# Hawkeye-FineGrained/Hawkeye

Hardware: NVIDIA H100
Metric: 448x448 images/sec, BCNN VGG-16 train step (fwd+CE+bwd+grad all-reduce+SGD), device-timed, max over ranks (higher is better)
Workload: dtype tf32 (fp32 storage, fp32 accumulate)

## Files before the change

hawkeye_b200/csrc/conv.cu:

```cuda
#include <stdlib.h>

#include "common.cuh"
#include "host.h"
#include "gemm.h"
#include "../../include/hawkeye_b200.h"

namespace hk {

__global__ void pack_weights_kernel(const float* __restrict__ W, float* __restrict__ Wf, float* __restrict__ Wd,
                                    int Cout, int Cin, int round) {
  const size_t n = (size_t)Cout * Cin * 9;
  for (size_t i = blockIdx.x * (size_t)blockDim.x + threadIdx.x; i < n; i += (size_t)gridDim.x * blockDim.x) {
    const int t = i % 9;
    const int ci = (i / 9) % Cin;
    const int co = i / ((size_t)9 * Cin);
    const float v = round ? tf32_round(W[i]) : W[i];
    if (Wf) Wf[((size_t)t * Cout + co) * Cin + ci] = v;
    if (Wd) Wd[((size_t)(8 - t) * Cin + ci) * Cout + co] = v;
  }
}
__global__ void unpack_wgrad_kernel(const float* __restrict__ dWp, float* __restrict__ dW, int Cout, int Cin, int accumulate) {
  const size_t n = (size_t)Cout * Cin * 9;
  for (size_t i = blockIdx.x * (size_t)blockDim.x + threadIdx.x; i < n; i += (size_t)gridDim.x * blockDim.x) {
    const int t = i % 9;
// ... 183 lines not shown
  const int co0 = blockIdx.y * BN;
  const int nchunk = a.Cin / 32;
  const int nk = 9 * nchunk;

  if (threadIdx.x == 0) {
    tma_prefetch_desc(&tmX);
    tma_prefetch_desc(&tmW);
    for (int s = 0; s < Cfg::STAGES; ++s) { mbar_init(&full[s], 1); mbar_init(&empty[s], 2); }
    fence_barrier_init();
  }
  __syncthreads();

  if (warp < 4) {
    regs_dealloc<56>();
    if (threadIdx.x == 0) {
      for (int kb = 0; kb < nk; ++kb) {
        const int s = kb % Cfg::STAGES;
        const uint32_t ph = (kb / Cfg::STAGES) & 1;
        const int tap = kb / nchunk, ck = kb - tap * nchunk;
        const int kh = tap / 3, kw = tap - kh * 3;
        mbar_wait(&empty[s], ph ^ 1);
        mbar_expect_tx(&full[s], Cfg::STAGE_BYTES);
        tma_load_4d(sA + s * Cfg::A_BYTES, &tmX, &full[s], ck * 32, w0 * a.stride + kw - 1, h0 * a.stride + kh - 1, n0);
        tma_load_3d(sB + s * Cfg::B_BYTES, &tmW, &full[s], ck * 32, co0, tap);
      }
    }
  } else {
    regs_alloc<224>();
    const int ct = threadIdx.x - 128;
    const int wg = ct >> 7;
    float acc[NACC];
    for (int kb = 0; kb < nk; ++kb) {
      const int s = kb % Cfg::STAGES;
      const uint32_t ph = (kb / Cfg::STAGES) & 1;
      mbar_wait(&full[s], ph);
      const uint64_t a_base = make_sdesc(smem_u32(sA + s * Cfg::A_BYTES + wg * 64 * 128));
      const uint64_t b_base = make_sdesc(smem_u32(sB + s * Cfg::B_BYTES));
      wgmma_fence();
#pragma unroll
      for (int ks = 0; ks < 4; ++ks) wgmma_tf32(acc, a_base + ks * 2, b_base + ks * 2, (kb | ks) != 0);
      wgmma_commit();
      wgmma_wait<1>();
      wgmma_keep(acc);
      if (kb > 0 && (ct & 127) == 0) mbar_arrive(&empty[(kb - 1) % Cfg::STAGES]);
    }
    wgmma_wait<0>();
    wgmma_keep(acc);
    conv_epilogue<BN>(a, acc, acc_tile, w0, h0, n0, co0, ct);
  }
}

static void pick_tile(int W, int H, int N, int target, int* TW, int* TH, int* TN) {
  int tw = 1;
  while (tw * 2 <= 16 && W % (tw * 2) == 0 && tw * 2 <= target) tw *= 2;
  int th = 1;
  while (th * 2 * tw <= target && H % (th * 2) == 0) th *= 2;
  int tn = target / (tw * th);
  *TW = tw; *TH = th; *TN = tn;
  (void)N;
}

static int make_act_map(CUtensorMap* tm, const float* X, int N, int H, int W, int C, int TW, int TH, int TN,
                        int stride = 1) {
  uint64_t dims[4] = {(uint64_t)C, (uint64_t)W, (uint64_t)H, (uint64_t)N};
  uint64_t strides[3] = {(uint64_t)C * 4, (uint64_t)W * C * 4, (uint64_t)H * W * C * 4};
  uint32_t box[4] = {32, (uint32_t)(TW * stride), (uint32_t)(TH * stride), (uint32_t)TN};
  uint32_t estr[4] = {1, (uint32_t)stride, (uint32_t)stride, 1};
  return make_tmap(tm, X, 4, dims, strides, box, stride > 1 ? estr : nullptr);
}

template <int BN>
static int launch_conv(const CUtensorMap& tmX, const CUtensorMap& tmW, const ConvArgs& a, cudaStream_t stream) {
  using Cfg = ConvCfg<BN>;
  if (int r = allow_dynamic_smem<conv3x3_igemm_kernel<BN>>(Cfg::SMEM, BN == 64 ? "conv<64>" : "conv<128>")) return r;
  dim3 grid(a.tiles_w * a.tiles_h * a.tiles_n, (a.Cout + BN - 1) / BN);
  conv3x3_igemm_kernel<BN><<<grid, CONV_THREADS, Cfg::SMEM, stream>>>(tmX, tmW, a);
  HK_LAUNCH_CHECK("conv3x3_igemm_kernel");
  return 0;
}

constexpr int CONV_V2_THREADS = 512;

enum { EPI_MAP = 0, EPI_UNPOOL = 1, EPI_FIRST_WGRAD = 2 };
constexpr int FW_HALO = 3 * 10 * 18;
constexpr int FW_HALO_BYTES = 2 * FW_HALO * 4;
struct FirstWgradArgs {
  const float* img;
  float* part;
};

__device__ __forceinline__ void mma_m16n8k8_tf32(float (&d)[4], const uint32_t (&a)[4], uint32_t b0, uint32_t b1) {
  asm volatile("mma.sync.aligned.m16n8k8.row.col.f32.tf32.tf32.f32 {%0, %1, %2, %3}, {%4, %5, %6, %7}, {%8, %9}, "
               "{%0, %1, %2, %3};\n"
               : "+f"(d[0]), "+f"(d[1]), "+f"(d[2]), "+f"(d[3])
               : "r"(a[0]), "r"(a[1]), "r"(a[2]), "r"(a[3]), "r"(b0), "r"(b1));
}

template <int BN, bool RESIDENT>
struct ConvV2Cfg {
  static constexpr int A_BYTES = 160 * 128;
  static constexpr int B_TILE = BN * 128;
  static constexpr int STAGE_BYTES = A_BYTES + (RESIDENT ? 0 : 3 * B_TILE);
  static constexpr int STAGES = RESIDENT ? 2 : (BN == 64 ? 3 : 2);
  static constexpr int WRES_BYTES = RESIDENT ? 18 * B_TILE : 0;
  static constexpr int PIECES = STAGES == 2 && !RESIDENT ? 3 : 1;
  static constexpr int STG_LD = BN + 8;
  static constexpr int STG_BYTES = 128 * STG_LD * 4;
  static constexpr int SMEM = STAGES * STAGE_BYTES + WRES_BYTES + 1024 + 256 + STG_BYTES;
};

template <int BN, bool RESIDENT, int TW, int EPI>
__global__ void __launch_bounds__(CONV_V2_THREADS, 1)
conv3x3_igemm_v2_kernel(const __grid_constant__ CUtensorMap tmX, const __grid_constant__ CUtensorMap tmW, ConvArgs a,
                        int n_ntiles, int total_tiles, FirstWgradArgs fw) {
  using Cfg = ConvV2Cfg<BN, RESIDENT>;
  static_assert(EPI != EPI_FIRST_WGRAD || (BN == 64 && RESIDENT && TW == 16), "conv1_1 weight gradient: 64 -> 64, 16 x 8");
  constexpr int NACC = BN / 2;
  constexpr int TN = 16 / TW;
  constexpr int WG_ROWS = TW == 16 ? 64 : 80;
  extern __shared__ uint8_t smem_raw[];
  uint8_t* smem = reinterpret_cast<uint8_t*>((reinterpret_cast<uintptr_t>(smem_raw) + 1023) & ~uintptr_t(1023));
  uint8_t* stages = smem;
  uint8_t* wres = smem + Cfg::STAGES * Cfg::STAGE_BYTES;
  uint64_t* full = reinterpret_cast<uint64_t*>(wres + Cfg::WRES_BYTES);
  uint64_t* empty = full + Cfg::STAGES * Cfg::PIECES;
  uint64_t* wbar = empty + Cfg::STAGES;
  uint64_t* stg_full = wbar + 1;
  uint64_t* stg_empty = wbar + 2;
  float* stg = reinterpret_cast<float*>(wres + Cfg::WRES_BYTES + 256);

  const int warp = threadIdx.x >> 5;
  const int nchunk = a.Cin / 32;
  const int nkb = nchunk * 3;

  if (threadIdx.x == 0) {
    tma_prefetch_desc(&tmX);
    tma_prefetch_desc(&tmW);
    for (int s = 0; s < Cfg::STAGES; ++s) mbar_init(&empty[s], 2);
    for (int i = 0; i < Cfg::STAGES * Cfg::PIECES; ++i) mbar_init(&full[i], 1);
    mbar_init(wbar, 1);
    mbar_init(stg_full, 256);
    mbar_init(stg_empty, 128);
    fence_barrier_init();
  }
  __syncthreads();

  if (warp >= 12 && EPI == EPI_MAP && a.P) {
    const int r = threadIdx.x - 384;
    int j = 0;
    for (int t = blockIdx.x; t < total_tiles; t += gridDim.x, ++j) {
      int pt = t / n_ntiles;
      const int co0 = (t - pt * n_ntiles) * BN;
      const int tw = pt % a.tiles_w; pt /= a.tiles_w;
      const int th = pt % a.tiles_h; pt /= a.tiles_h;
      mbar_wait(stg_full, j & 1);
      const int w = tw * TW + (r & (TW - 1)), h = th * 8 + ((r / TW) & 7), n = pt * TN + r / (TW * 8);
      const bool valid = TN == 1 || n < a.N;
      const size_t pix = ((size_t)n * a.H + h) * a.W + w;
#pragma unroll 1
      for (int c = 0; c < BN / 32; ++c) {
        float v[32];
        const float4* src = reinterpret_cast<const float4*>(stg + r * Cfg::STG_LD + c * 32);
#pragma unroll
        for (int k = 0; k < 8; ++k) {
          const float4 q = src[k];
          v[4 * k] = q.x; v[4 * k + 1] = q.y; v[4 * k + 2] = q.z; v[4 * k + 3] = q.w;
        }
        if (c == BN / 32 - 1) mbar_arrive(stg_empty);
        epi_chunk<true>(a, v, w, h, n, pix, co0 + c * 32, valid);
      }
    }
  } else if (warp >= 12) {
    const int e = threadIdx.x - 384;
    const int ew = e >> 5, sub = (e >> 3) & 3, u4 = (e & 7) * 4;
    const int p0 = ew * 32 + sub;
    const int eoff0 = (TW == 16 ? (p0 >> 4) * a.W + (p0 & 15) : ((p0 >> 6) * a.H + ((p0 >> 3) & 7)) * a.W + (p0 & 7)) * a.Cout + u4;
    const int erow = a.W * a.Cout, e4 = 4 * a.Cout;
    auto eoff = [&](int k) { return eoff0 + (k / (TW / 4)) * erow + (k % (TW / 4)) * e4; };
    const float* srow = stg + (ew * 32 + sub) * Cfg::STG_LD + u4;
    auto tile_org = [&](int t, size_t& org, int& co0) {
      co0 = (t % n_ntiles) * BN;
      int pt = t / n_ntiles;
      const int tw = pt % a.tiles_w; pt /= a.tiles_w;
      const int th = pt % a.tiles_h; pt /= a.tiles_h;
      org = (((size_t)pt * TN * a.H + th * 8) * a.W + tw * TW) * a.Cout;
      return pt * TN + (TW == 16 ? 0 : ew >> 1) < a.N;
    };
    auto tile_pos = [&](int t, int& tw, int& th, int& tn) {
      int pt = t / n_ntiles;
      tw = pt % a.tiles_w; pt /= a.tiles_w;
      th = pt % a.tiles_h; tn = pt / a.tiles_h;
    };
    const int frow = 2 * a.W * a.Cout;
    const int uoff0 = (TW == 16 ? 2 * (p0 >> 4) * frow + 2 * (p0 & 15) * a.Cout
                                : ((p0 >> 6) * 2 * a.H + 2 * ((p0 >> 3) & 7)) * frow + 2 * (p0 & 7) * a.Cout) + u4;
    auto uoff = [&](int k) { return uoff0 + (k / (TW / 4)) * 2 * frow + (k % (TW / 4)) * 8 * a.Cout; };
    float* halo = stg + 128 * Cfg::STG_LD;
    float dacc[4][4] = {};
    const int lane = e & 31, g = lane >> 2, tq = lane & 3;
    int hoff[4];
#pragma unroll
    for (int nt = 0; nt < 4; ++nt) {
      const int jj = 8 * nt + g;
      hoff[nt] = jj < 27 ? (jj / 9) * 180 + (jj % 9 / 3) * 18 + jj % 3 : 0;
    }
    int co0 = 0, j = 0;
    size_t org = 0;
    for (int t = blockIdx.x; t < total_tiles; t += gridDim.x, ++j) {
      const bool valid = tile_org(t, org, co0);
      if constexpr (EPI == EPI_FIRST_WGRAD) {
        int tw, th, tn;
        tile_pos(t, tw, th, tn);
        float* hb = halo + (j & 1) * FW_HALO;
        for (int i = e; i < FW_HALO; i += 128) {
          const int ci = i / 180, hh = th * 8 - 1 + i / 18 % 10, ww = tw * 16 - 1 + i % 18;
          hb[i] = hh >= 0 && hh < a.H && ww >= 0 && ww < a.W
                      ? tf32_round(__ldg(fw.img + (((size_t)tn * 3 + ci) * a.H + hh) * a.W + ww)) : 0.f;
        }
      }
      mbar_wait(stg_full, j & 1);
#pragma unroll
      for (int c = 0; c < BN / 32; ++c) {
        float4 v[8];
#pragma unroll
        for (int k = 0; k < 8; ++k) v[k] = *reinterpret_cast<const float4*>(srow + 4 * k * Cfg::STG_LD + c * 32);
        if (EPI != EPI_FIRST_WGRAD && c == BN / 32 - 1) mbar_arrive(stg_empty);
        const int co = co0 + c * 32;
        const bool live = valid && co < a.Cout;
        if (live) {
          if (a.bias) {
            const float4 b = __ldg(reinterpret_cast<const float4*>(a.bias + co + u4));
#pragma unroll
            for (int k = 0; k < 8; ++k) { v[k].x += b.x; v[k].y += b.y; v[k].z += b.z; v[k].w += b.w; }
          }
          if (a.relu) {
#pragma unroll
            for (int k = 0; k < 8; ++k) {
              v[k].x = fmaxf(v[k].x, 0.f); v[k].y = fmaxf(v[k].y, 0.f);
              v[k].z = fmaxf(v[k].z, 0.f); v[k].w = fmaxf(v[k].w, 0.f);
            }
          }
          if (a.mask) {
            float4 mk[8];
#pragma unroll
            for (int k = 0; k < 8; ++k) mk[k] = __ldcs(reinterpret_cast<const float4*>(a.mask + org + co + eoff(k)));
#pragma unroll
            for (int k = 0; k < 8; ++k) {
              v[k].x = mk[k].x > 0.f ? v[k].x : 0.f; v[k].y = mk[k].y > 0.f ? v[k].y : 0.f;
              v[k].z = mk[k].z > 0.f ? v[k].z : 0.f; v[k].w = mk[k].w > 0.f ? v[k].w : 0.f;
            }
          }
          if constexpr (EPI == EPI_MAP) {
#pragma unroll
            for (int k = 0; k < 8; ++k)
              __stcs(reinterpret_cast<float4*>(a.Y + org + co + eoff(k)),
                     make_float4(tf32_round(v[k].x), tf32_round(v[k].y), tf32_round(v[k].z), tf32_round(v[k].w)));
          } else if constexpr (EPI == EPI_UNPOOL) {
            int tw, th, tn;
            tile_pos(t, tw, th, tn);
            float* dst = a.Y + (((size_t)tn * TN * 2 * a.H + th * 16) * 2 * a.W + tw * 2 * TW) * a.Cout + co;
            uint32_t cd[8];
#pragma unroll
            for (int k = 0; k < 8; ++k) cd[k] = __ldcs(reinterpret_cast<const unsigned int*>(a.code + org + co + eoff(k)));
#pragma unroll
            for (int k = 0; k < 8; ++k) {
              const float4 q = make_float4((cd[k] & 4u) ? tf32_round(v[k].x) : 0.f, (cd[k] & (4u << 8)) ? tf32_round(v[k].y) : 0.f,
                                           (cd[k] & (4u << 16)) ? tf32_round(v[k].z) : 0.f,
                                           (cd[k] & (4u << 24)) ? tf32_round(v[k].w) : 0.f);
              float* o = dst + uoff(k);
#pragma unroll
              for (int pos = 0; pos < 4; ++pos)
                __stcs(reinterpret_cast<float4*>(o + (pos >> 1) * frow + (pos & 1) * a.Cout),
                       make_float4((cd[k] & 3u) == (uint32_t)pos ? q.x : 0.f, (cd[k] >> 8 & 3u) == (uint32_t)pos ? q.y : 0.f,
                                   (cd[k] >> 16 & 3u) == (uint32_t)pos ? q.z : 0.f,
                                   (cd[k] >> 24 & 3u) == (uint32_t)pos ? q.w : 0.f));
            }
          } else {
#pragma unroll
            for (int k = 0; k < 8; ++k)
              *reinterpret_cast<float4*>(stg + (ew * 32 + sub + 4 * k) * Cfg::STG_LD + u4 + c * 32) =
                  make_float4(tf32_round(v[k].x), tf32_round(v[k].y), tf32_round(v[k].z), tf32_round(v[k].w));
          }
        }
      }
      if constexpr (EPI == EPI_FIRST_WGRAD) {
        named_bar(1, 128);
        const float* hb = halo + (j & 1) * FW_HALO;
        const float* arow = stg + tq * Cfg::STG_LD + 16 * ew + g;
#pragma unroll 4
        for (int ks = 0; ks < 16; ++ks) {
          const float* ap = arow + 8 * ks * Cfg::STG_LD;
          const uint32_t af[4] = {__float_as_uint(ap[0]), __float_as_uint(ap[8]), __float_as_uint(ap[4 * Cfg::STG_LD]),
                                  __float_as_uint(ap[4 * Cfg::STG_LD + 8])};
          const int hp = (ks >> 1) * 18 + 8 * (ks & 1) + tq;
#pragma unroll
          for (int nt = 0; nt < 4; ++nt) {
            float b0 = hb[hoff[nt] + hp], b1 = hb[hoff[nt] + hp + 4];
            if (nt == 3 && g >= 3) b0 = b1 = g == 3 ? 1.f : 0.f;
            mma_m16n8k8_tf32(dacc[nt], af, __float_as_uint(b0), __float_as_uint(b1));
          }
        }
        mbar_arrive(stg_empty);
      }
    }
    if constexpr (EPI == EPI_FIRST_WGRAD) {
      float* dst = fw.part + (size_t)blockIdx.x * 64 * 32;
#pragma unroll
      for (int nt = 0; nt < 4; ++nt)
#pragma unroll
        for (int i = 0; i < 4; ++i) dst[(16 * ew + g + 8 * (i >> 1)) * 32 + 8 * nt + 2 * tq + (i & 1)] = dacc[nt][i];
    }
  } else if (warp < 4) {
    if (threadIdx.x == 0) {
      if (RESIDENT) {
        mbar_expect_tx(wbar, Cfg::WRES_BYTES);
        for (int tap = 0; tap < 9; ++tap)
          for (int ck = 0; ck < 2; ++ck) tma_load_3d(wres + (tap * 2 + ck) * Cfg::B_TILE, &tmW, wbar, ck * 32, 0, tap);
      }
      int kbg = 0;
      for (int t = blockIdx.x; t < total_tiles; t += gridDim.x) {
        const int nt = t % n_ntiles;
        int pt = t / n_ntiles;
        const int tw = pt % a.tiles_w; pt /= a.tiles_w;
        const int th = pt % a.tiles_h; pt /= a.tiles_h;
        const int w0 = tw * TW, h0 = th * 8, n0 = pt * TN, co0 = nt * BN;
        for (int kb = 0; kb < nkb; ++kb, ++kbg) {
          const int s = kbg % Cfg::STAGES;
          const uint32_t ph = (kbg / Cfg::STAGES) & 1;
          const int ck = kb / 3, kw = kb - ck * 3;
          mbar_wait(&empty[s], ph ^ 1);
          uint64_t* f = full + s * Cfg::PIECES;
          uint8_t* st = stages + s * Cfg::STAGE_BYTES;
          mbar_expect_tx(&f[0], Cfg::PIECES == 3 ? Cfg::A_BYTES + Cfg::B_TILE : Cfg::STAGE_BYTES);
          tma_load_4d(st, &tmX, &f[0], ck * 32, w0 + kw - 1, h0 - 1, n0);
          if (!RESIDENT) {
#pragma unroll
            for (int kh = 0; kh < 3; ++kh) {
              uint64_t* fk = &f[Cfg::PIECES == 3 ? kh : 0];
              if (Cfg::PIECES == 3 && kh > 0) mbar_expect_tx(fk, Cfg::B_TILE);
              tma_load_3d(st + Cfg::A_BYTES + kh * Cfg::B_TILE, &tmW, fk, ck * 32, co0, kh * 3 + kw);
            }
          }
        }
      }
    }
  } else {
    const int ct = threadIdx.x - 128;
    const int wg = ct >> 7;
    if (RESIDENT) mbar_wait(wbar, 0);
    float acc[NACC];
#pragma unroll
    for (int i = 0; i < NACC; ++i) acc[i] = 0.f;
    float* frag = stg + (wg * 64 + ((ct >> 5) & 3) * 16 + ((ct & 31) >> 2)) * Cfg::STG_LD + 2 * (ct & 3);
    int kbg = 0, j = 0;
    for (int t = blockIdx.x; t < total_tiles; t += gridDim.x, ++j) {
      for (int kb = 0; kb < nkb; ++kb, ++kbg) {
        const int s = kbg % Cfg::STAGES;
        const int ck = kb / 3, kw = kb - ck * 3;
        const uint32_t ph = (kbg / Cfg::STAGES) & 1;
        const uint32_t a_addr = smem_u32(stages + s * Cfg::STAGE_BYTES) + wg * WG_ROWS * 128;
#pragma unroll
        for (int kh = 0; kh < 3; ++kh) {
          if (kh < Cfg::PIECES) {
            mbar_wait(&full[s * Cfg::PIECES + kh], ph);
            wgmma_fence();
          }
          const uint32_t b_addr = RESIDENT ? smem_u32(wres + ((kh * 3 + kw) * 2 + ck) * Cfg::B_TILE)
                                           : smem_u32(stages + s * Cfg::STAGE_BYTES + Cfg::A_BYTES + kh * Cfg::B_TILE);
          const uint64_t ad = make_sdesc(a_addr + kh * TW * 128), bd = make_sdesc(b_addr);
#pragma unroll
          for (int ks = 0; ks < 4; ++ks) wgmma_tf32(acc, ad + ks * 2, bd + ks * 2, (kb | kh | ks) != 0);
          if (kh >= 3 - Cfg::PIECES) wgmma_commit();
          if (kh == 3 - Cfg::PIECES) {
            wgmma_wait<1>();
            wgmma_keep(acc);
            if (kb > 0 && (ct & 127) == 0) mbar_arrive(&empty[(kbg - 1) % Cfg::STAGES]);
          }
        }
      }
      wgmma_wait<0>();
      wgmma_keep(acc);
      if ((ct & 127) == 0) mbar_arrive(&empty[(kbg - 1) % Cfg::STAGES]);
      mbar_wait(stg_empty, (j & 1) ^ 1);
#pragma unroll
      for (int i = 0; i < NACC / 4; ++i) {
        *reinterpret_cast<float2*>(frag + 8 * i) = make_float2(acc[4 * i], acc[4 * i + 1]);
        *reinterpret_cast<float2*>(frag + 8 * Cfg::STG_LD + 8 * i) = make_float2(acc[4 * i + 2], acc[4 * i + 3]);
      }
      mbar_arrive(stg_full);
    }
  }
}

template <int BN, bool RESIDENT, int TW, int EPI = EPI_MAP>
static int launch_conv_v2(const float* x, const float* wp, ConvArgs a, int N, int H, int W, cudaStream_t stream,
                          FirstWgradArgs fw = {}) {
  using Cfg = ConvV2Cfg<BN, RESIDENT>;
  constexpr int SMEM = Cfg::SMEM + (EPI == EPI_FIRST_WGRAD ? FW_HALO_BYTES : 0);
  static_assert(SMEM <= 232448, "conv_v2: dynamic shared memory above the sm_90 opt-in limit");
  if (int r = allow_dynamic_smem<conv3x3_igemm_v2_kernel<BN, RESIDENT, TW, EPI>>(SMEM, BN == 64 ? "conv_v2<64>" : "conv_v2<128>"))
    return r;
  a.TW = TW; a.TH = 8; a.TN = 16 / TW;
  a.tiles_w = W / TW; a.tiles_h = H / 8; a.tiles_n = (N + a.TN - 1) / a.TN;
  const int n_ntiles = (a.Cout + BN - 1) / BN;
  const long long total = (long long)a.tiles_w * a.tiles_h * a.tiles_n * n_ntiles;
  HK_REQUIRE(total < (1ll << 31), HK_ERR_UNSUPPORTED, "conv3x3: too many tiles");
  HK_REQUIRE((long long)H * W * a.Cout < (1ll << 30), HK_ERR_UNSUPPORTED, "conv3x3: map too large");
  CUtensorMap tmX, tmW;
  int r;
  {
    uint64_t dims[4] = {(uint64_t)a.Cin, (uint64_t)W, (uint64_t)H, (uint64_t)N};
    uint64_t strides[3] = {(uint64_t)a.Cin * 4, (uint64_t)W * a.Cin * 4, (uint64_t)H * W * a.Cin * 4};
    uint32_t box[4] = {32, (uint32_t)TW, 10, (uint32_t)a.TN};
    if ((r = make_tmap(&tmX, x, 4, dims, strides, box))) return r;
  }
  {
    uint64_t dims[3] = {(uint64_t)a.Cin, (uint64_t)a.Cout, 9};
    uint64_t strides[2] = {(uint64_t)a.Cin * 4, (uint64_t)a.Cin * a.Cout * 4};
    uint32_t box[3] = {32, (uint32_t)BN, 1};
    if ((r = make_tmap(&tmW, wp, 3, dims, strides, box))) return r;
  }
  const int sms = num_sms();
  const int grid = total < sms ? (int)total : sms;
  conv3x3_igemm_v2_kernel<BN, RESIDENT, TW, EPI><<<grid, CONV_V2_THREADS, SMEM, stream>>>(tmX, tmW, a, n_ntiles, (int)total, fw);
  HK_LAUNCH_CHECK("conv3x3_igemm_v2_kernel");
  return 0;
}

template <int TW, int EPI = EPI_MAP>
static int launch_conv_v2(const float* x, const float* wp, const ConvArgs& a, int N, int H, int W, cudaStream_t stream) {
  if (a.Cin == 64 && a.Cout == 64) return launch_conv_v2<64, true, TW, EPI>(x, wp, a, N, H, W, stream);
  if (a.Cout <= 64) return launch_conv_v2<64, false, TW, EPI>(x, wp, a, N, H, W, stream);
  return launch_conv_v2<128, false, TW, EPI>(x, wp, a, N, H, W, stream);
}

static int conv3x3_igemm_1x(const float* x, const float* wp, const float* bias, const float* mask, const float* addend,
                            float* y, int N, int H, int W, int Cin, int Cout, int relu, cudaStream_t stream, int stride,
                            int no_round, float* pooled = nullptr, unsigned char* code = nullptr,
                            int pool_nchw = 0);

int conv3x3_igemm(const float* x, const float* wp, const float* bias, const float* mask, float* y, int N, int H, int W,
                  int Cin, int Cout, int relu, cudaStream_t stream, int stride = 1) {
  if (!precise()) return conv3x3_igemm_1x(x, wp, bias, mask, nullptr, y, N, H, W, Cin, Cout, relu, stream, stride, 0);
  HK_REQUIRE(x && wp && y, HK_ERR_ARG, "conv3x3: null pointer");
  const size_t nx = (size_t)N * H * W * Cin, nw = (size_t)9 * Cout * Cin;
  Scratch sx(2 * nx * sizeof(float), stream), sw(2 * nw * sizeof(float), stream);
  HK_REQUIRE(sx.p && sw.p, HK_ERR_DRIVER, "conv3x3 (precise): cudaMallocAsync of the operand halves failed");
  float *xh = sx.f(), *xl = xh + nx, *wh = sw.f(), *wl = wh + nw;
  int r;
  if ((r = tf32_split(x, xh, xl, nx, stream))) return r;
  if ((r = tf32_split(wp, wh, wl, nw, stream))) return r;
  if ((r = conv3x3_igemm_1x(xh, wl, nullptr, nullptr, nullptr, y, N, H, W, Cin, Cout, 0, stream, stride, 1))) return r;
  if ((r = conv3x3_igemm_1x(xl, wh, nullptr, nullptr, y, y, N, H, W, Cin, Cout, 0, stream, stride, 1))) return r;
  return conv3x3_igemm_1x(xh, wh, bias, mask, y, y, N, H, W, Cin, Cout, relu, stream, stride, 1);
}

static int conv3x3_igemm_1x(const float* x, const float* wp, const float* bias, const float* mask, const float* addend,
                            float* y, int N, int H, int W, int Cin, int Cout, int relu, cudaStream_t stream, int stride,
                            int no_round, float* pooled, unsigned char* code, int pool_nchw) {
  const int Hin = H, Win = W;
  if (stride == 2) {
    HK_REQUIRE(H % 2 == 0 && W % 2 == 0, HK_ERR_UNSUPPORTED, "conv3x3 stride 2: even H/W required");
    H /= 2; W /= 2;
  }
  HK_REQUIRE(x && wp && (y || pooled), HK_ERR_ARG, "conv3x3: null pointer");
  HK_REQUIRE(Cin % 32 == 0 && Cout % 32 == 0, HK_ERR_UNSUPPORTED, "conv3x3: Cin=%d Cout=%d must be multiples of 32",
             Cin, Cout);
  HK_REQUIRE(aligned16(x) && aligned16(wp) && (!y || aligned16(y)) && (!mask || aligned16(mask)), HK_ERR_ALIGN,
             "conv3x3: pointer not 16-byte aligned");
  if (pooled)
    HK_REQUIRE(stride == 1 && H % 2 == 0 && W % 2 == 0 && aligned16(pooled) && (!code || aligned16(code)), HK_ERR_UNSUPPORTED,
               "conv3x3 + pool: even H/W, stride 1 and 16-byte aligned outputs required");
  ConvArgs a = {};
  a.P = pooled; a.code = code; a.pool_nchw = pool_nchw;
  a.Y = y; a.bias = bias; a.mask = mask; a.N = N; a.H = H; a.W = W; a.Cin = Cin; a.Cout = Cout; a.relu = relu;
  a.stride = stride;
  a.addend = addend; a.no_round = no_round;
  if (!no_round && stride == 1 && W % 8 == 0 && H % 8 == 0) {
    if (W % 16 == 0) return launch_conv_v2<16>(x, wp, a, N, H, W, stream);
    return launch_conv_v2<8>(x, wp, a, N, H, W, stream);
  }
  pick_tile(W, H, N, 128, &a.TW, &a.TH, &a.TN);
  HK_REQUIRE(!pooled || (a.TW >= 2 && a.TH >= 2), HK_ERR_UNSUPPORTED, "conv3x3 + pool: pixel tile %dx%d", a.TW, a.TH);
  a.tiles_w = (W + a.TW - 1) / a.TW; a.tiles_h = (H + a.TH - 1) / a.TH; a.tiles_n = (N + a.TN - 1) / a.TN;
  HK_REQUIRE((long long)a.tiles_w * a.tiles_h * a.tiles_n < (1ll << 31), HK_ERR_UNSUPPORTED, "conv3x3: grid too large");
  CUtensorMap tmX, tmW;
  int r;
  if ((r = make_act_map(&tmX, x, N, Hin, Win, Cin, a.TW, a.TH, a.TN, stride))) return r;
  const int BN = Cout <= 64 ? 64 : 128;
  {
    uint64_t dims[3] = {(uint64_t)Cin, (uint64_t)Cout, 9};
    uint64_t strides[2] = {(uint64_t)Cin * 4, (uint64_t)Cin * Cout * 4};
    uint32_t box[3] = {32, (uint32_t)BN, 1};
    if ((r = make_tmap(&tmW, wp, 3, dims, strides, box))) return r;
  }
  if (BN == 64) return launch_conv<64>(tmX, tmW, a, stream);
  return launch_conv<128>(tmX, tmW, a, stream);
}

struct WgradArgs {
  float* dWp;
  float* db;
  int N, H, W, Cin, Cout;
  int TW, TH, TN, tiles_w, tiles_h, tiles_n;
  int total_tiles, per;
};

constexpr int WG_THREADS = 4 * 128;
constexpr int WG_PRODUCER_REGS = 56, WG_CONSUMER_REGS = 152;
static_assert(128 * WG_PRODUCER_REGS + 3 * 128 * WG_CONSUMER_REGS <= 65536, "wgrad register budget");
constexpr int WG_STAGES = 3;
constexpr int WG_KP = 64;
constexpr int WG_RAW_ROWS = 120;
constexpr int WG_RAW_BYTES = WG_RAW_ROWS * 128;
// ... 569 lines not shown
  if (sub >= lanes_per_c) return;
  const size_t per = (npix + gridDim.x - 1) / gridDim.x;
  const size_t p0 = blockIdx.x * per, p1 = (p0 + per < npix) ? p0 + per : npix;
  for (int cc = c; cc < C; cc += (blockDim.x < C ? blockDim.x : C)) {
    float s = 0.f;
    for (size_t p = p0 + sub; p < p1; p += lanes_per_c) s += dy[p * C + cc];
    atomicAdd(db + cc, s);
  }
}

}

using namespace hk;

extern "C" {

int hk_conv3x3_pack_weights(const float* w, float* w_fwd, float* w_dgrad, int Cout, int Cin, void* stream) {
  HK_REQUIRE(w && (w_fwd || w_dgrad), HK_ERR_ARG, "hk_conv3x3_pack_weights: null pointer");
  pack_weights_kernel<<<grid_1d((size_t)Cout * Cin * 9, 256), 256, 0, (cudaStream_t)stream>>>(w, w_fwd, w_dgrad, Cout, Cin,
                                                                                              precise() ? 0 : 1);
  HK_LAUNCH_CHECK("pack_weights_kernel");
  return 0;
}

int hk_conv3x3_fwd(const float* x, const float* w_packed, const float* bias, float* y, int N, int H, int W, int Cin,
                   int Cout, int relu, void* stream) {
  return conv3x3_igemm(x, w_packed, bias, nullptr, y, N, H, W, Cin, Cout, relu, (cudaStream_t)stream);
}

int hk_conv3x3_fwd_pool(const float* x, const float* w_packed, const float* bias, float* pooled, unsigned char* code, int N,
                        int H, int W, int Cin, int Cout, int out_nchw, void* stream) {
  HK_REQUIRE(!precise(), HK_ERR_UNSUPPORTED, "hk_conv3x3_fwd_pool: not available in 3xTF32 mode (use conv + pool)");
  HK_REQUIRE(pooled, HK_ERR_ARG, "hk_conv3x3_fwd_pool: null output");
  return conv3x3_igemm_1x(x, w_packed, bias, nullptr, nullptr, nullptr, N, H, W, Cin, Cout, 1, (cudaStream_t)stream, 1,
                          0, pooled, code, out_nchw);
}

int hk_conv3x3_s2_fwd(const float* x, const float* w_packed, const float* bias, float* y, int N, int H, int W, int Cin,
                      int Cout, int relu, void* stream) {
  return conv3x3_igemm(x, w_packed, bias, nullptr, y, N, H, W, Cin, Cout, relu, (cudaStream_t)stream, 2);
}

int hk_conv3x3_dgrad(const float* dy, const float* w_dgrad_packed, const float* relu_mask_act, float* dx, int N, int H,
                     int W, int Cin, int Cout, void* stream) {
  return conv3x3_igemm(dy, w_dgrad_packed, nullptr, relu_mask_act, dx, N, H, W, Cout, Cin, 0, (cudaStream_t)stream);
}

int hk_conv3x3_dgrad_unpool(const float* dy, const float* w_dgrad_packed, const unsigned char* code, float* dx_full, int N,
                            int H, int W, int Cin, int Cout, void* stream) {
  HK_REQUIRE(!precise(), HK_ERR_UNSUPPORTED, "hk_conv3x3_dgrad_unpool: not available in 3xTF32 mode");
  HK_REQUIRE(dy && w_dgrad_packed && code && dx_full, HK_ERR_ARG, "hk_conv3x3_dgrad_unpool: null pointer");
  HK_REQUIRE(N > 0 && H > 0 && W > 0, HK_ERR_ARG, "hk_conv3x3_dgrad_unpool: empty map");
  HK_REQUIRE(Cin % 32 == 0 && Cout % 32 == 0, HK_ERR_UNSUPPORTED,
             "hk_conv3x3_dgrad_unpool: Cin=%d Cout=%d must be multiples of 32", Cin, Cout);
  HK_REQUIRE(H % 8 == 0 && W % 8 == 0, HK_ERR_UNSUPPORTED, "hk_conv3x3_dgrad_unpool: %dx%d map is not a multiple of 8x8",
             H, W);
  HK_REQUIRE(4ll * H * W * Cin < (1ll << 31), HK_ERR_UNSUPPORTED, "hk_conv3x3_dgrad_unpool: map too large");
  HK_REQUIRE(aligned16(dy) && aligned16(w_dgrad_packed) && aligned16(code) && aligned16(dx_full), HK_ERR_ALIGN,
             "hk_conv3x3_dgrad_unpool: pointer not 16-byte aligned");
  ConvArgs a = {};
  a.Y = dx_full; a.code = const_cast<unsigned char*>(code);
  a.N = N; a.H = H; a.W = W; a.Cin = Cout; a.Cout = Cin; a.stride = 1;
  if (W % 16 == 0) return launch_conv_v2<16, EPI_UNPOOL>(dy, w_dgrad_packed, a, N, H, W, (cudaStream_t)stream);
  return launch_conv_v2<8, EPI_UNPOOL>(dy, w_dgrad_packed, a, N, H, W, (cudaStream_t)stream);
}

size_t hk_conv3x3_dgrad_first_wgrad_workspace_bytes(void) { return (size_t)num_sms() * 64 * 32 * sizeof(float); }

int hk_conv3x3_dgrad_first_wgrad_acc(const float* dy, const float* w_dgrad_packed, const float* relu_mask_act,
                                     const float* x_nchw, float* dw1, float* db1, int N, int H, int W, int Cin, int Cout,
                                     void* workspace, size_t workspace_bytes, int accumulate, void* stream_) {
  cudaStream_t stream = (cudaStream_t)stream_;
  HK_REQUIRE(!precise(), HK_ERR_UNSUPPORTED, "hk_conv3x3_dgrad_first_wgrad: not available in 3xTF32 mode");
  HK_REQUIRE(dy && w_dgrad_packed && x_nchw && dw1, HK_ERR_ARG, "hk_conv3x3_dgrad_first_wgrad: null pointer");
  HK_REQUIRE(N > 0 && H > 0 && W > 0, HK_ERR_ARG, "hk_conv3x3_dgrad_first_wgrad: empty map");
  HK_REQUIRE(Cin == 64 && Cout == 64, HK_ERR_UNSUPPORTED, "hk_conv3x3_dgrad_first_wgrad: Cin=%d Cout=%d (64 -> 64 only)",
             Cin, Cout);
  HK_REQUIRE(W % 16 == 0 && H % 8 == 0, HK_ERR_UNSUPPORTED,
             "hk_conv3x3_dgrad_first_wgrad: %dx%d map is not tiled by 16x8", H, W);
  HK_REQUIRE(aligned16(dy) && aligned16(w_dgrad_packed) && (!relu_mask_act || aligned16(relu_mask_act)), HK_ERR_ALIGN,
             "hk_conv3x3_dgrad_first_wgrad: pointer not 16-byte aligned");
  HK_REQUIRE(workspace && workspace_bytes >= hk_conv3x3_dgrad_first_wgrad_workspace_bytes(), HK_ERR_WORKSPACE,
             "hk_conv3x3_dgrad_first_wgrad: workspace too small");
  const long long tiles = (long long)(W / 16) * (H / 8) * N;
  HK_REQUIRE(tiles < (1ll << 31), HK_ERR_UNSUPPORTED, "hk_conv3x3_dgrad_first_wgrad: too many tiles");
  float* part = static_cast<float*>(workspace);
  ConvArgs a = {};
  a.mask = relu_mask_act;
  a.N = N; a.H = H; a.W = W; a.Cin = Cout; a.Cout = Cin; a.stride = 1;
  int r = launch_conv_v2<64, true, 16, EPI_FIRST_WGRAD>(dy, w_dgrad_packed, a, N, H, W, stream, FirstWgradArgs{x_nchw, part});
  if (r) return r;
  const int G = tiles < num_sms() ? (int)tiles : num_sms();
  if ((r = sum_splits(part, G, 64 * 32, 64, 27, 32, dw1, 27, nullptr, accumulate, stream))) return r;
  if (!db1) return 0;
  return sum_splits(part + 27, G, 64 * 32, 64, 1, 32, db1, 1, nullptr, accumulate, stream);
}

size_t hk_conv3x3_wgrad_workspace_bytes(int Cin, int Cout) { return (size_t)9 * Cin * Cout * sizeof(float); }

int hk_conv3x3_wgrad_acc(const float* x, const float* dy, float* dw, float* db, int N, int H, int W, int Cin, int Cout,
                         void* workspace, size_t workspace_bytes, int accumulate, void* stream_) {
  cudaStream_t stream = (cudaStream_t)stream_;
  HK_REQUIRE(workspace && workspace_bytes >= hk_conv3x3_wgrad_workspace_bytes(Cin, Cout), HK_ERR_WORKSPACE,
             "hk_conv3x3_wgrad: workspace too small");
  HK_REQUIRE(dw, HK_ERR_ARG, "hk_conv3x3_wgrad: null dw");
  float* dwp = static_cast<float*>(workspace);
  int r = conv3x3_wgrad(x, dy, dwp, db, N, H, W, Cin, Cout, stream, !accumulate);
  if (r) return r;
  unpack_wgrad_kernel<<<grid_1d((size_t)Cout * Cin * 9, 256), 256, 0, stream>>>(dwp, dw, Cout, Cin, accumulate ? 1 : 0);
  HK_LAUNCH_CHECK("unpack_wgrad_kernel");
  return 0;
}

int hk_conv3x3_wgrad(const float* x, const float* dy, float* dw, float* db, int N, int H, int W, int Cin, int Cout,
                     void* workspace, size_t workspace_bytes, void* stream_) {
  return hk_conv3x3_wgrad_acc(x, dy, dw, db, N, H, W, Cin, Cout, workspace, workspace_bytes, 0, stream_);
}

size_t hk_conv3x3_first_fwd_workspace_bytes(int N, int H, int W, int Cout) {
  return ((size_t)N * H * W * 32 + (size_t)Cout * 32) * sizeof(float);
}

int hk_conv3x3_first_fwd(const float* x_nchw, const float* w, const float* bias, float* y_nhwc, int N, int H, int W,
                         int Cout, void* workspace, size_t workspace_bytes, void* stream_) {
  cudaStream_t stream = (cudaStream_t)stream_;
  HK_REQUIRE(x_nchw && w && y_nhwc, HK_ERR_ARG, "hk_conv3x3_first_fwd: null pointer");
  HK_REQUIRE(Cout % 4 == 0 && Cout <= 256, HK_ERR_UNSUPPORTED, "hk_conv3x3_first_fwd: Cout=%d unsupported", Cout);
  HK_REQUIRE(workspace && workspace_bytes >= hk_conv3x3_first_fwd_workspace_bytes(N, H, W, Cout), HK_ERR_WORKSPACE,
             "hk_conv3x3_first_fwd: workspace too small");
  const long long P = (long long)N * H * W;
  HK_REQUIRE(P < (1ll << 31), HK_ERR_UNSUPPORTED, "hk_conv3x3_first_fwd: too many pixels");
  float* x27 = static_cast<float*>(workspace);
  float* w27 = x27 + (size_t)P * 32;
  const int round = precise() ? 0 : 1;
  im2col_first_kernel<<<grid_1d((size_t)P, 128), 128, 0, stream>>>(x_nchw, x27, N, H, W, round);
  HK_LAUNCH_CHECK("im2col_first_kernel");
  pack_first_weights_kernel<<<(Cout * 32 + 127) / 128, 128, 0, stream>>>(w, bias, w27, Cout, round);
  HK_LAUNCH_CHECK("pack_first_weights_kernel");
  GemmEpi e = {};
  e.C = y_nhwc; e.ldc = Cout; e.alpha = 1.f;
  e.relu = 3;
  return gemm_tf32(x27, 0, 32, 0, w27, 0, 32, 0, e, (int)P, Cout, 32, 1, stream);
}

static int first_wgrad_splits(long long P) {
  for (int S = 592; S > 1; --S)
    if (P % S == 0) return S;
  return 1;
}

size_t hk_conv3x3_first_wgrad_workspace_bytes(int N, int H, int W, int Cout) {
  return (size_t)first_wgrad_splits((long long)N * H * W) * Cout * 32 * sizeof(float);
}

int hk_conv3x3_first_wgrad_acc(const float* x27, const float* dy_nhwc, float* dw, float* db, int N, int H, int W, int Cout,
                               void* workspace, size_t workspace_bytes, int accumulate, void* stream_);
int hk_conv3x3_first_wgrad(const float* x27, const float* dy_nhwc, float* dw, float* db, int N, int H, int W,
                           int Cout, void* workspace, size_t workspace_bytes, void* stream_) {
  return hk_conv3x3_first_wgrad_acc(x27, dy_nhwc, dw, db, N, H, W, Cout, workspace, workspace_bytes, 0, stream_);
}
int hk_conv3x3_first_wgrad_acc(const float* x27, const float* dy_nhwc, float* dw, float* db, int N, int H, int W, int Cout,
                               void* workspace, size_t workspace_bytes, int accumulate, void* stream_) {
  cudaStream_t stream = (cudaStream_t)stream_;
  HK_REQUIRE(x27 && dy_nhwc && dw, HK_ERR_ARG, "hk_conv3x3_first_wgrad: null pointer");
  HK_REQUIRE(Cout % 4 == 0 && Cout <= 128, HK_ERR_UNSUPPORTED, "hk_conv3x3_first_wgrad: Cout=%d unsupported", Cout);
  HK_REQUIRE(workspace && workspace_bytes >= hk_conv3x3_first_wgrad_workspace_bytes(N, H, W, Cout), HK_ERR_WORKSPACE,
             "hk_conv3x3_first_wgrad: workspace too small");
  const long long P = (long long)N * H * W;
  const int S = first_wgrad_splits(P);
  float* part = static_cast<float*>(workspace);
  int r = gemm_splitk(dy_nhwc, 1, Cout, x27, 1, 32, Cout, 32, P, S, part, dw, 27, 27, nullptr, accumulate, stream);
  if (r || !db) return r;
  return sum_splits(part + 27, S, (long long)Cout * 32, Cout, 1, 32, db, 1, nullptr, accumulate, stream);
// ... 83 lines not shown
```

Baseline: 826.7.

## Use 16x16 pixel tiles with swapped wgmma operands for 64-channel TW=16 convs

For BN=64 with 16-wide tiles, the conv kernel now processes a 16x16 (256-pixel) tile by swapping operands so the weights become the wgmma A operand and pixels the N dimension. It streams weights instead of keeping them resident, uses two stages, enlarges the halo and staging buffer, and runs the epilogue in two 128-pixel halves. The first-layer fused dgrad+wgrad path is moved onto this larger tile. The aim is to halve per-tile overhead and halo reloads and to use wider wgmma instructions, at the cost of more shared memory, a transposed staging write pattern with more bank traffic, and handling partial tiles when H is not a multiple of 16.

```diff
diff --git a/hawkeye_b200/csrc/conv.cu b/hawkeye_b200/csrc/conv.cu
--- a/hawkeye_b200/csrc/conv.cu
+++ b/hawkeye_b200/csrc/conv.cu
@@ -289,7 +289,8 @@
 constexpr int CONV_V2_THREADS = 512;
 
 enum { EPI_MAP = 0, EPI_UNPOOL = 1, EPI_FIRST_WGRAD = 2 };
-constexpr int FW_HALO = 3 * 10 * 18;
+constexpr int FW_HALO_CH = 18 * 18;
+constexpr int FW_HALO = 3 * FW_HALO_CH;
 constexpr int FW_HALO_BYTES = 2 * FW_HALO * 4;
 struct FirstWgradArgs {
   const float* img;
@@ -303,16 +304,21 @@
                : "r"(a[0]), "r"(a[1]), "r"(a[2]), "r"(a[3]), "r"(b0), "r"(b1));
 }
 
-template <int BN, bool RESIDENT>
+template <int BN, bool RESIDENT, int TW>
 struct ConvV2Cfg {
-  static constexpr int A_BYTES = 160 * 128;
+  static constexpr bool SWAP = BN == 64 && TW == 16;
+  static_assert(!(SWAP && RESIDENT), "the 256-pixel tile streams its weights");
+  static constexpr int TH = SWAP ? 16 : 8, TN = 16 / TW;
+  static constexpr int PIX = TW * TH * TN;
+  static constexpr int NACC = BN * PIX / 256;
+  static constexpr int A_BYTES = (TH + 2) * TW * TN * 128;
   static constexpr int B_TILE = BN * 128;
   static constexpr int STAGE_BYTES = A_BYTES + (RESIDENT ? 0 : 3 * B_TILE);
-  static constexpr int STAGES = RESIDENT ? 2 : (BN == 64 ? 3 : 2);
+  static constexpr int STAGES = RESIDENT ? 2 : (BN == 64 && !SWAP ? 3 : 2);
   static constexpr int WRES_BYTES = RESIDENT ? 18 * B_TILE : 0;
   static constexpr int PIECES = STAGES == 2 && !RESIDENT ? 3 : 1;
-  static constexpr int STG_LD = BN + 8;
-  static constexpr int STG_BYTES = 128 * STG_LD * 4;
+  static constexpr int STG_LD = SWAP ? BN + 4 : BN + 8;
+  static constexpr int STG_BYTES = PIX * STG_LD * 4;
   static constexpr int SMEM = STAGES * STAGE_BYTES + WRES_BYTES + 1024 + 256 + STG_BYTES;
 };
 
@@ -320,11 +326,12 @@
 __global__ void __launch_bounds__(CONV_V2_THREADS, 1)
 conv3x3_igemm_v2_kernel(const __grid_constant__ CUtensorMap tmX, const __grid_constant__ CUtensorMap tmW, ConvArgs a,
                         int n_ntiles, int total_tiles, FirstWgradArgs fw) {
-  using Cfg = ConvV2Cfg<BN, RESIDENT>;
-  static_assert(EPI != EPI_FIRST_WGRAD || (BN == 64 && RESIDENT && TW == 16), "conv1_1 weight gradient: 64 -> 64, 16 x 8");
-  constexpr int NACC = BN / 2;
-  constexpr int TN = 16 / TW;
-  constexpr int WG_ROWS = TW == 16 ? 64 : 80;
+  using Cfg = ConvV2Cfg<BN, RESIDENT, TW>;
+  static_assert(EPI != EPI_FIRST_WGRAD || Cfg::SWAP, "conv1_1 weight gradient: 64 -> 64, 16 x 16");
+  constexpr int NACC = Cfg::NACC;
+  constexpr int TH = Cfg::TH, TN = Cfg::TN;
+  constexpr int NHALF = Cfg::PIX / 128;
+  constexpr int WG_ROWS = Cfg::SWAP ? 128 : TW == 16 ? 64 : 80;
   extern __shared__ uint8_t smem_raw[];
   uint8_t* smem = reinterpret_cast<uint8_t*>((reinterpret_cast<uintptr_t>(smem_raw) + 1023) & ~uintptr_t(1023));
   uint8_t* stages = smem;
@@ -353,7 +360,7 @@
   __syncthreads();
 
   if (warp >= 12 && EPI == EPI_MAP && a.P) {
-    const int r = threadIdx.x - 384;
+    const int r0 = threadIdx.x - 384;
     int j = 0;
     for (int t = blockIdx.x; t < total_tiles; t += gridDim.x, ++j) {
       int pt = t / n_ntiles;
@@ -361,20 +368,24 @@
       const int tw = pt % a.tiles_w; pt /= a.tiles_w;
       const int th = pt % a.tiles_h; pt /= a.tiles_h;
       mbar_wait(stg_full, j & 1);
-      const int w = tw * TW + (r & (TW - 1)), h = th * 8 + ((r / TW) & 7), n = pt * TN + r / (TW * 8);
-      const bool valid = TN == 1 || n < a.N;
-      const size_t pix = ((size_t)n * a.H + h) * a.W + w;
+#pragma unroll
+      for (int hf = 0; hf < NHALF; ++hf) {
+        const int r = r0 + 128 * hf;
+        const int w = tw * TW + (r & (TW - 1)), h = th * TH + (r / TW) % TH, n = pt * TN + r / (TW * TH);
+        const bool valid = (TN == 1 || n < a.N) && h < a.H;
+        const size_t pix = ((size_t)n * a.H + h) * a.W + w;
 #pragma unroll 1
-      for (int c = 0; c < BN / 32; ++c) {
-        float v[32];
-        const float4* src = reinterpret_cast<const float4*>(stg + r * Cfg::STG_LD + c * 32);
-#pragma unroll
-        for (int k = 0; k < 8; ++k) {
-          const float4 q = src[k];
-          v[4 * k] = q.x; v[4 * k + 1] = q.y; v[4 * k + 2] = q.z; v[4 * k + 3] = q.w;
+        for (int c = 0; c < BN / 32; ++c) {
+          float v[32];
+          const float4* src = reinterpret_cast<const float4*>(stg + r * Cfg::STG_LD + c * 32);
+#pragma unroll
+          for (int k = 0; k < 8; ++k) {
+            const float4 q = src[k];
+            v[4 * k] = q.x; v[4 * k + 1] = q.y; v[4 * k + 2] = q.z; v[4 * k + 3] = q.w;
+          }
+          if (hf == NHALF - 1 && c == BN / 32 - 1) mbar_arrive(stg_empty);
+          epi_chunk<true>(a, v, w, h, n, pix, co0 + c * 32, valid);
         }
-        if (c == BN / 32 - 1) mbar_arrive(stg_empty);
-        epi_chunk<true>(a, v, w, h, n, pix, co0 + c * 32, valid);
       }
     }
   } else if (warp >= 12) {
@@ -385,12 +396,13 @@
     const int erow = a.W * a.Cout, e4 = 4 * a.Cout;
     auto eoff = [&](int k) { return eoff0 + (k / (TW / 4)) * erow + (k % (TW / 4)) * e4; };
     const float* srow = stg + (ew * 32 + sub) * Cfg::STG_LD + u4;
-    auto tile_org = [&](int t, size_t& org, int& co0) {
+    auto tile_org = [&](int t, size_t& org, int& co0, int& h0) {
       co0 = (t % n_ntiles) * BN;
       int pt = t / n_ntiles;
       const int tw = pt % a.tiles_w; pt /= a.tiles_w;
       const int th = pt % a.tiles_h; pt /= a.tiles_h;
-      org = (((size_t)pt * TN * a.H + th * 8) * a.W + tw * TW) * a.Cout;
+      h0 = th * TH;
+      org = (((size_t)pt * TN * a.H + h0) * a.W + tw * TW) * a.Cout;
       return pt * TN + (TW == 16 ? 0 : ew >> 1) < a.N;
     };
     auto tile_pos = [&](int t, int& tw, int& th, int& tn) {
@@ -402,38 +414,49 @@
     const int uoff0 = (TW == 16 ? 2 * (p0 >> 4) * frow + 2 * (p0 & 15) * a.Cout
                                 : ((p0 >> 6) * 2 * a.H + 2 * ((p0 >> 3) & 7)) * frow + 2 * (p0 & 7) * a.Cout) + u4;
     auto uoff = [&](int k) { return uoff0 + (k / (TW / 4)) * 2 * frow + (k % (TW / 4)) * 8 * a.Cout; };
-    float* halo = stg + 128 * Cfg::STG_LD;
+    float* halo = stg + Cfg::PIX * Cfg::STG_LD;
     float dacc[4][4] = {};
     const int lane = e & 31, g = lane >> 2, tq = lane & 3;
     int hoff[4];
 #pragma unroll
     for (int nt = 0; nt < 4; ++nt) {
       const int jj = 8 * nt + g;
-      hoff[nt] = jj < 27 ? (jj / 9) * 180 + (jj % 9 / 3) * 18 + jj % 3 : 0;
-    }
-    int co0 = 0, j = 0;
+      hoff[nt] = jj < 27 ? (jj / 9) * FW_HALO_CH + (jj % 9 / 3) * 18 + jj % 3 : 0;
+    }
+    int co0 = 0, h0 = 0, j = 0;
     size_t org = 0;
     for (int t = blockIdx.x; t < total_tiles; t += gridDim.x, ++j) {
-      const bool valid = tile_org(t, org, co0);
+      const bool valid = tile_org(t, org, co0, h0);
       if constexpr (EPI == EPI_FIRST_WGRAD) {
         int tw, th, tn;
         tile_pos(t, tw, th, tn);
         float* hb = halo + (j & 1) * FW_HALO;
-        for (int i = e; i < FW_HALO; i += 128) {
-          const int ci = i / 180, hh = th * 8 - 1 + i / 18 % 10, ww = tw * 16 - 1 + i % 18;
-          hb[i] = hh >= 0 && hh < a.H && ww >= 0 && ww < a.W
-                      ? tf32_round(__ldg(fw.img + (((size_t)tn * 3 + ci) * a.H + hh) * a.W + ww)) : 0.f;
+        constexpr int FW_PER_THREAD = (FW_HALO + 127) / 128;
+        float hv[FW_PER_THREAD];
+#pragma unroll
+        for (int k = 0; k < FW_PER_THREAD; ++k) {
+          const int i = e + 128 * k;
+          const int ci = i / FW_HALO_CH, hh = h0 - 1 + i / 18 % 18, ww = tw * 16 - 1 + i % 18;
+          hv[k] = i < FW_HALO && hh >= 0 && hh < a.H && ww >= 0 && ww < a.W
+                      ? __ldg(fw.img + (((size_t)tn * 3 + ci) * a.H + hh) * a.W + ww) : 0.f;
         }
+#pragma unroll
+        for (int k = 0; k < FW_PER_THREAD; ++k)
+          if (e + 128 * k < FW_HALO) hb[e + 128 * k] = tf32_round(hv[k]);
       }
       mbar_wait(stg_full, j & 1);
+#pragma unroll
+      for (int hf = 0; hf < NHALF; ++hf)
 #pragma unroll
       for (int c = 0; c < BN / 32; ++c) {
         float4 v[8];
-#pragma unroll
-        for (int k = 0; k < 8; ++k) v[k] = *reinterpret_cast<const float4*>(srow + 4 * k * Cfg::STG_LD + c * 32);
-        if (EPI != EPI_FIRST_WGRAD && c == BN / 32 - 1) mbar_arrive(stg_empty);
+        const int hs = hf * 128 * Cfg::STG_LD;
+        const int ho = hf * 8 * erow;
+#pragma unroll
+        for (int k = 0; k < 8; ++k) v[k] = *reinterpret_cast<const float4*>(srow + hs + 4 * k * Cfg::STG_LD + c * 32);
+        if (EPI != EPI_FIRST_WGRAD && hf == NHALF - 1 && c == BN / 32 - 1) mbar_arrive(stg_empty);
         const int co = co0 + c * 32;
-        const bool live = valid && co < a.Cout;
+        const bool live = valid && co < a.Cout && (NHALF == 1 || h0 + 8 * hf < a.H);
         if (live) {
           if (a.bias) {
             const float4 b = __ldg(reinterpret_cast<const float4*>(a.bias + co + u4));
@@ -450,7 +473,7 @@
           if (a.mask) {
             float4 mk[8];
 #pragma unroll
-            for (int k = 0; k < 8; ++k) mk[k] = __ldcs(reinterpret_cast<const float4*>(a.mask + org + co + eoff(k)));
+            for (int k = 0; k < 8; ++k) mk[k] = __ldcs(reinterpret_cast<const float4*>(a.mask + org + ho + co + eoff(k)));
 #pragma unroll
             for (int k = 0; k < 8; ++k) {
               v[k].x = mk[k].x > 0.f ? v[k].x : 0.f; v[k].y = mk[k].y > 0.f ? v[k].y : 0.f;
@@ -460,15 +483,15 @@
           if constexpr (EPI == EPI_MAP) {
 #pragma unroll
             for (int k = 0; k < 8; ++k)
-              __stcs(reinterpret_cast<float4*>(a.Y + org + co + eoff(k)),
+              __stcs(reinterpret_cast<float4*>(a.Y + org + ho + co + eoff(k)),
                      make_float4(tf32_round(v[k].x), tf32_round(v[k].y), tf32_round(v[k].z), tf32_round(v[k].w)));
           } else if constexpr (EPI == EPI_UNPOOL) {
             int tw, th, tn;
             tile_pos(t, tw, th, tn);
-            float* dst = a.Y + (((size_t)tn * TN * 2 * a.H + th * 16) * 2 * a.W + tw * 2 * TW) * a.Cout + co;
+            float* dst = a.Y + (((size_t)tn * TN * 2 * a.H + th * 2 * TH) * 2 * a.W + tw * 2 * TW) * a.Cout + co + hf * 16 * frow;
             uint32_t cd[8];
 #pragma unroll
-            for (int k = 0; k < 8; ++k) cd[k] = __ldcs(reinterpret_cast<const unsigned int*>(a.code + org + co + eoff(k)));
+            for (int k = 0; k < 8; ++k) cd[k] = __ldcs(reinterpret_cast<const unsigned int*>(a.code + org + ho + co + eoff(k)));
 #pragma unroll
             for (int k = 0; k < 8; ++k) {
               const float4 q = make_float4((cd[k] & 4u) ? tf32_round(v[k].x) : 0.f, (cd[k] & (4u << 8)) ? tf32_round(v[k].y) : 0.f,
@@ -485,7 +508,7 @@
           } else {
 #pragma unroll
             for (int k = 0; k < 8; ++k)
-              *reinterpret_cast<float4*>(stg + (ew * 32 + sub + 4 * k) * Cfg::STG_LD + u4 + c * 32) =
+              *reinterpret_cast<float4*>(stg + hs + (ew * 32 + sub + 4 * k) * Cfg::STG_LD + u4 + c * 32) =
                   make_float4(tf32_round(v[k].x), tf32_round(v[k].y), tf32_round(v[k].z), tf32_round(v[k].w));
           }
         }
@@ -494,8 +517,9 @@
         named_bar(1, 128);
         const float* hb = halo + (j & 1) * FW_HALO;
         const float* arow = stg + tq * Cfg::STG_LD + 16 * ew + g;
+        const int nks = 2 * min(TH, a.H - h0);
 #pragma unroll 4
-        for (int ks = 0; ks < 16; ++ks) {
+        for (int ks = 0; ks < nks; ++ks) {
           const float* ap = arow + 8 * ks * Cfg::STG_LD;
           const uint32_t af[4] = {__float_as_uint(ap[0]), __float_as_uint(ap[8]), __float_as_uint(ap[4 * Cfg::STG_LD]),
                                   __float_as_uint(ap[4 * Cfg::STG_LD + 8])};
@@ -530,7 +554,7 @@
         int pt = t / n_ntiles;
         const int tw = pt % a.tiles_w; pt /= a.tiles_w;
         const int th = pt % a.tiles_h; pt /= a.tiles_h;
-        const int w0 = tw * TW, h0 = th * 8, n0 = pt * TN, co0 = nt * BN;
+        const int w0 = tw * TW, h0 = th * TH, n0 = pt * TN, co0 = nt * BN;
         for (int kb = 0; kb < nkb; ++kb, ++kbg) {
           const int s = kbg % Cfg::STAGES;
           const uint32_t ph = (kbg / Cfg::STAGES) & 1;
@@ -558,23 +582,25 @@
     float acc[NACC];
 #pragma unroll
     for (int i = 0; i < NACC; ++i) acc[i] = 0.f;
-    float* frag = stg + (wg * 64 + ((ct >> 5) & 3) * 16 + ((ct & 31) >> 2)) * Cfg::STG_LD + 2 * (ct & 3);
+    const int r0 = ((ct >> 5) & 3) * 16 + ((ct & 31) >> 2), c0 = 2 * (ct & 3);
+    float* frag = Cfg::SWAP ? stg + (wg * 128 + c0) * Cfg::STG_LD + r0 : stg + (wg * 64 + r0) * Cfg::STG_LD + c0;
     int kbg = 0, j = 0;
     for (int t = blockIdx.x; t < total_tiles; t += gridDim.x, ++j) {
       for (int kb = 0; kb < nkb; ++kb, ++kbg) {
         const int s = kbg % Cfg::STAGES;
         const int ck = kb / 3, kw = kb - ck * 3;
         const uint32_t ph = (kbg / Cfg::STAGES) & 1;
-        const uint32_t a_addr = smem_u32(stages + s * Cfg::STAGE_BYTES) + wg * WG_ROWS * 128;
+        const uint32_t p_addr = smem_u32(stages + s * Cfg::STAGE_BYTES) + wg * WG_ROWS * 128;
 #pragma unroll
         for (int kh = 0; kh < 3; ++kh) {
           if (kh < Cfg::PIECES) {
             mbar_wait(&full[s * Cfg::PIECES + kh], ph);
             wgmma_fence();
           }
-          const uint32_t b_addr = RESIDENT ? smem_u32(wres + ((kh * 3 + kw) * 2 + ck) * Cfg::B_TILE)
+          const uint32_t w_addr = RESIDENT ? smem_u32(wres + ((kh * 3 + kw) * 2 + ck) * Cfg::B_TILE)
                                            : smem_u32(stages + s * Cfg::STAGE_BYTES + Cfg::A_BYTES + kh * Cfg::B_TILE);
-          const uint64_t ad = make_sdesc(a_addr + kh * TW * 128), bd = make_sdesc(b_addr);
+          const uint64_t pd = make_sdesc(p_addr + kh * TW * 128), wd = make_sdesc(w_addr);
+          const uint64_t ad = Cfg::SWAP ? wd : pd, bd = Cfg::SWAP ? pd : wd;
 #pragma unroll
           for (int ks = 0; ks < 4; ++ks) wgmma_tf32(acc, ad + ks * 2, bd + ks * 2, (kb | kh | ks) != 0);
           if (kh >= 3 - Cfg::PIECES) wgmma_commit();
@@ -591,8 +617,14 @@
       mbar_wait(stg_empty, (j & 1) ^ 1);
 #pragma unroll
       for (int i = 0; i < NACC / 4; ++i) {
-        *reinterpret_cast<float2*>(frag + 8 * i) = make_float2(acc[4 * i], acc[4 * i + 1]);
-        *reinterpret_cast<float2*>(frag + 8 * Cfg::STG_LD + 8 * i) = make_float2(acc[4 * i + 2], acc[4 * i + 3]);
+        if constexpr (Cfg::SWAP) {
+          float* f = frag + 8 * i * Cfg::STG_LD;
+          f[0] = acc[4 * i]; f[Cfg::STG_LD] = acc[4 * i + 1];
+          f[8] = acc[4 * i + 2]; f[Cfg::STG_LD + 8] = acc[4 * i + 3];
+        } else {
+          *reinterpret_cast<float2*>(frag + 8 * i) = make_float2(acc[4 * i], acc[4 * i + 1]);
+          *reinterpret_cast<float2*>(frag + 8 * Cfg::STG_LD + 8 * i) = make_float2(acc[4 * i + 2], acc[4 * i + 3]);
+        }
       }
       mbar_arrive(stg_full);
     }
@@ -602,13 +634,13 @@
 template <int BN, bool RESIDENT, int TW, int EPI = EPI_MAP>
 static int launch_conv_v2(const float* x, const float* wp, ConvArgs a, int N, int H, int W, cudaStream_t stream,
                           FirstWgradArgs fw = {}) {
-  using Cfg = ConvV2Cfg<BN, RESIDENT>;
+  using Cfg = ConvV2Cfg<BN, RESIDENT, TW>;
   constexpr int SMEM = Cfg::SMEM + (EPI == EPI_FIRST_WGRAD ? FW_HALO_BYTES : 0);
   static_assert(SMEM <= 232448, "conv_v2: dynamic shared memory above the sm_90 opt-in limit");
   if (int r = allow_dynamic_smem<conv3x3_igemm_v2_kernel<BN, RESIDENT, TW, EPI>>(SMEM, BN == 64 ? "conv_v2<64>" : "conv_v2<128>"))
     return r;
-  a.TW = TW; a.TH = 8; a.TN = 16 / TW;
-  a.tiles_w = W / TW; a.tiles_h = H / 8; a.tiles_n = (N + a.TN - 1) / a.TN;
+  a.TW = TW; a.TH = Cfg::TH; a.TN = Cfg::TN;
+  a.tiles_w = W / TW; a.tiles_h = (H + a.TH - 1) / a.TH; a.tiles_n = (N + a.TN - 1) / a.TN;
   const int n_ntiles = (a.Cout + BN - 1) / BN;
   const long long total = (long long)a.tiles_w * a.tiles_h * a.tiles_n * n_ntiles;
   HK_REQUIRE(total < (1ll << 31), HK_ERR_UNSUPPORTED, "conv3x3: too many tiles");
@@ -618,7 +650,7 @@
   {
     uint64_t dims[4] = {(uint64_t)a.Cin, (uint64_t)W, (uint64_t)H, (uint64_t)N};
     uint64_t strides[3] = {(uint64_t)a.Cin * 4, (uint64_t)W * a.Cin * 4, (uint64_t)H * W * a.Cin * 4};
-    uint32_t box[4] = {32, (uint32_t)TW, 10, (uint32_t)a.TN};
+    uint32_t box[4] = {32, (uint32_t)TW, (uint32_t)a.TH + 2, (uint32_t)a.TN};
     if ((r = make_tmap(&tmX, x, 4, dims, strides, box))) return r;
   }
   {
@@ -636,7 +668,8 @@
 
 template <int TW, int EPI = EPI_MAP>
 static int launch_conv_v2(const float* x, const float* wp, const ConvArgs& a, int N, int H, int W, cudaStream_t stream) {
-  if (a.Cin == 64 && a.Cout == 64) return launch_conv_v2<64, true, TW, EPI>(x, wp, a, N, H, W, stream);
+  if constexpr (TW == 8)
+    if (a.Cin == 64 && a.Cout == 64) return launch_conv_v2<64, true, TW, EPI>(x, wp, a, N, H, W, stream);
   if (a.Cout <= 64) return launch_conv_v2<64, false, TW, EPI>(x, wp, a, N, H, W, stream);
   return launch_conv_v2<128, false, TW, EPI>(x, wp, a, N, H, W, stream);
 }
@@ -1372,13 +1405,14 @@
              "hk_conv3x3_dgrad_first_wgrad: pointer not 16-byte aligned");
   HK_REQUIRE(workspace && workspace_bytes >= hk_conv3x3_dgrad_first_wgrad_workspace_bytes(), HK_ERR_WORKSPACE,
              "hk_conv3x3_dgrad_first_wgrad: workspace too small");
-  const long long tiles = (long long)(W / 16) * (H / 8) * N;
-  HK_REQUIRE(tiles < (1ll << 31), HK_ERR_UNSUPPORTED, "hk_conv3x3_dgrad_first_wgrad: too many tiles");
+  HK_REQUIRE((long long)(W / 16) * (H / 8) * N < (1ll << 31), HK_ERR_UNSUPPORTED,
+             "hk_conv3x3_dgrad_first_wgrad: too many tiles");
+  const long long tiles = (long long)(W / 16) * ((H + 15) / 16) * N;
   float* part = static_cast<float*>(workspace);
   ConvArgs a = {};
   a.mask = relu_mask_act;
   a.N = N; a.H = H; a.W = W; a.Cin = Cout; a.Cout = Cin; a.stride = 1;
-  int r = launch_conv_v2<64, true, 16, EPI_FIRST_WGRAD>(dy, w_dgrad_packed, a, N, H, W, stream, FirstWgradArgs{x_nchw, part});
+  int r = launch_conv_v2<64, false, 16, EPI_FIRST_WGRAD>(dy, w_dgrad_packed, a, N, H, W, stream, FirstWgradArgs{x_nchw, part});
   if (r) return r;
   const int G = tiles < num_sms() ? (int)tiles : num_sms();
   if ((r = sum_splits(part, G, 64 * 32, 64, 27, 32, dw1, 27, nullptr, accumulate, stream))) return r;
```

New measurement: 846.6 (median of 6 runs). 1.02x the previous value.
